# tsai0507/PolishPathPlanning

Hardware: AMD Instinct MI355X
Metric: polishing waypoints/sec for 1M-pt cloud, 256 slices; path L2 err vs ref (higher is better)
Workload: dtype f32; 1 GPU; cfg2_1m_s256; points_per_workpiece=999912, slices=256, waypoints_per_workpiece=25908, workpieces=1, batch_per_gpu=1, parallelism=single GPU, pairing=kd, walk=center_int (connect), dynamic_adjustment=False, handles_taking_turns=3

## Files before the change

### polishpathplanning_amd/csrc/ppp_engine.hip

```cpp
#include "ppp_kernels.h"
#ifdef PPP_SINGLE_TU
#include "ppp_window.h"
#endif
#include "ppp_handle.h"
#include "ppp_gather.h"
#include <atomic>
#include <cerrno>
#include <fcntl.h>
#include <thread>
#include <unistd.h>
#ifndef PPP_NN_HINT_SPACINGS
#define PPP_NN_HINT_SPACINGS 3.0
#endif
#ifndef PPP_SLAB_PTS
#define PPP_SLAB_PTS 832
#endif
#ifndef PPP_PPT8_FROM
#define PPP_PPT8_FROM 500000
#endif
#ifndef WIN_SLICE_WAVES_PER_CU
#define WIN_SLICE_WAVES_PER_CU 16
#endif
#ifndef PPP_WIN_PPT8_FROM
#define PPP_WIN_PPT8_FROM 1200000
// ... 410 lines not shown
static void win_args_throughput(const ppp_handle h, WinArgs &A)
{
    A.NBc = h->win_NBc_thr; A.NB = WIN_CLASSES * A.NBc;
    const float yr = h->h_mx[1] - h->h_mn[1];
    A.yscale = yr > 0.f ? (float)A.NBc / yr : 0.f;
}

static int enqueue_window_gen(ppp_handle h)
{
    WinArgs A = win_args(h);
    const bool thr = win_throughput_launch(h, A.g_slice);
    if (thr) win_args_throughput(h, A);
    const size_t scat_lds = win_scatter_lds_bytes(A.S, h->win_ppt, h->win_scat_threads, h->win_staged);
    if (h->win_scat_threads != WSC_T) {
        const int rcn = with_narrow_scatter(h->win_scat_threads, h->win_ppt, [&](auto ppt, auto st) -> int {
            LAUNCH(h, "k_win_scatter", (k_win_scatter<decltype(ppt)::value, false, decltype(st)::value>), A.g_scatter, decltype(st)::value, scat_lds, A);
            return PPP_OK;
        });
        if (rcn) return rcn;
    }
    else if (h->win_staged && h->win_ppt == 8) LAUNCH(h, "k_win_scatter", (k_win_scatter<8, true>), A.g_scatter, WSC_T, scat_lds, A);
    else if (h->win_staged) LAUNCH(h, "k_win_scatter", (k_win_scatter<4, true>), A.g_scatter, WSC_T, scat_lds, A);
    else if (h->win_ppt == 8) LAUNCH(h, "k_win_scatter", (k_win_scatter<8, false>), A.g_scatter, WSC_T, scat_lds, A);
    else if (h->win_ppt == 2) LAUNCH(h, "k_win_scatter", (k_win_scatter<2, false>), A.g_scatter, WSC_T, scat_lds, A);
    else LAUNCH(h, "k_win_scatter", (k_win_scatter<4, false>), A.g_scatter, WSC_T, scat_lds, A);
    const int T = h->win_threads;
    const size_t lds = win_slice_lds_for(h, A.NBc);
    const int extra = tuning_env("PPP_WIN_NO_VERIFY") ? 0 : 1;
    return with_block_size(T, [&](auto bs) -> int {
        LAUNCH(h, "k_win_slice", k_win_slice<decltype(bs)::value>, A.g_slice + extra, T, lds, A);
        return PPP_OK;
    });
}
static int enqueue_window_finish(ppp_handle h)
{
    const WinArgs A = win_args(h);
    LAUNCH(h, "k_win_finish", k_win_finish, A.g_finish, SMF_T, sizeof(int) * ((size_t)A.nkept + 2), A);
    return PPP_OK;
}

static int make_plan(ppp_handle h)
{
    if (!h->have_cloud) return fail(h, PPP_ERR_ARG, "no cloud set");
    h->pass.withdraw_plan();
    h->drop_graph();
    const int n = (int)h->n;
    int S = h->h_nvalid ? ppp_slice_walk(h->P.walk, h->h_mn[0], h->h_mx[0], h->P.tool_radius, nullptr, 0) : 0;
    if (S >= PPP_WALK_HARD_MAX) return fail(h, PPP_ERR_CAPACITY, "slice walk does not terminate");
    h->sb = std::min(std::max(0, h->P.slice_begin), S);
    h->se = (h->P.slice_end <= 0 || h->P.slice_end > S) ? S : h->P.slice_end;
    h->ranged = S > 0 && (h->sb > 0 || h->se < S);
    h->incl_lo = -INFINITY; h->incl_hi = INFINITY;
    h->n_range = h->h_nvalid;
    if (h->ranged) {
        if (h->sb >= h->se) { h->incl_lo = INFINITY; h->incl_hi = -INFINITY; h->n_range = 0; }
        else {
            std::vector<float> px((size_t)S);
            ppp_slice_walk(h->P.walk, h->h_mn[0], h->h_mx[0], h->P.tool_radius, px.data(), S);
            h->incl_lo = (float)((int)px[h->sb] - 2) - h->P.range_margin;
            h->incl_hi = (float)((int)px[h->se - 1] + 2) + h->P.range_margin;
            const double range = (double)h->h_mx[0] - (double)h->h_mn[0];
            const double part = std::min((double)h->incl_hi, (double)h->h_mx[0]) - std::max((double)h->incl_lo, (double)h->h_mn[0]);
            h->n_range = range > 0 ? (int)std::min((double)h->h_nvalid, std::max(0.0, part / range) * h->h_nvalid * 1.05 + 64) : h->h_nvalid;
        }
    }
    h->use_part = false; h->n_part = 0;
    if (h->part_given) {
        if (!h->ranged && !(h->part_lo == -INFINITY && h->part_hi == INFINITY))
            return fail(h, PPP_ERR_ARG, "a part-only cloud (ppp_set_cloud_part) needs a slice range: set slice_begin / slice_end");
// ... 902 lines not shown
    const SlabGeom G = slab_geom(h);
    const SlabArgs A = slab_args(h, G);
    int rc = enqueue_index(h, G, A);
    if (rc) return rc;
    if (h->P.pairing == PPP_PAIR_KD) {
        LAUNCH(h, "k_slice_kd", k_slice_kd<false>, A.g_slice, G.slice_threads(h->num_cus), G.slice_lds(), A);
        if (h->big_path) LAUNCH(h, "k_slice_kd_arena", k_slice_kd<true>, A.g_slice, SLICE_KD_T, 0, A);
    } else {
        LAUNCH(h, "k_slice", k_slice, A.g_slice, K_SLICE_T, G.brute_lds(), A);
        if (h->big_path) LAUNCH(h, "k_slice_brute_arena", k_slice_brute_arena, A.g_slice, 1024, 0, A);
    }
    if (h->P.dynamic_adjustment) {
        int rc2 = enqueue_dynamic(h);
        if (rc2) return rc2;
    }
    h->pass.gen_enqueued(false);
    if (h->chain_calls) return PPP_OK;
    return enqueue_meta_copy(h);
}

int enqueue_finish(ppp_handle h, const SlabArgs &A)
{
    LAUNCH(h, "k_smooth_solve", k_smooth_solve, A.g_smooth, SMF_T, 0, A);
    return enqueue_meta_copy(h);
}

int ppp_get_path_async(ppp_handle h)
{
    if (!h) return PPP_ERR_ARG;
    HIPCHK(h, hipSetDevice(h->device));
    { int rcs = settle_enqueue_only(h); if (rcs) return rcs; }
    if (!h->pass.gen_done()) return fail(h, PPP_ERR_ARG, "call ppp_gen_path_async first");
    if (h->win_path) {
        int rcw = enqueue_window_finish(h);
        if (rcw) return rcw;
        h->pass.path_enqueued(!h->ranged, true);
        h->pass.meta_will_arrive(MetaAt::pinned());
        return PPP_OK;
    }
    const SlabGeom G = slab_geom(h);
    const SlabArgs A = slab_args(h, G);
    PoseBack PB;
    memset(&PB, 0, sizeof(PB));
    if (h->aligned) {
        if (h->ranged) return fail(h, PPP_ERR_UNSUPPORTED, "Alignment with a slice range");
        if (!h->back || !h->back->pass.index_built()) return fail(h, PPP_ERR_ARG, "aligned cloud without its sensor-frame index");
        PB.sorted4 = h->back->sorted4.p; PB.slab_start = h->back->slab_start.p; PB.slab_xmin = h->back->slab_xmin.p; PB.slab_xmax = h->back->slab_xmax.p;
        PB.m = h->back->meta.p; PB.ytab = h->back->slab_ytab.p;
        for (int r = 0; r < 3; ++r) for (int c = 0; c < 4; ++c) PB.inv[r][c] = h->invTA[r][c];
        LAUNCH(h, "k_pose<aligned>", (k_pose<true, POSE_T>), A.g_pose, G.pose_threads, G.pose_lds, A, PB);
    } else {
        const int rcp = with_block_size(G.pose_threads, [&](auto bs) -> int {
            LAUNCH(h, "k_pose", (k_pose<false, decltype(bs)::value>), A.g_pose, G.pose_threads, G.pose_lds, A, PB);
            return PPP_OK;
        });
        if (rcp) return rcp;
    }
    h->pass.path_enqueued(false, false);
    if (!h->ranged) {
        int rc = enqueue_finish(h, A);
        if (rc) return rc;
        h->pass.path_enqueued(true, false);
        return PPP_OK;
    }
    return enqueue_meta_copy(h);
}

int ppp_finish_path_async(ppp_handle h, const float *pre6_dev, size_t W, const int *counts, size_t nkept)
{
// ... 519 lines not shown
}

int ppp_get_tail_index(ppp_handle h, int *tail, size_t cap, size_t *n)
{
    int rc = ensure_ready(h, true, true);
    if (rc) return rc;
    if (!h->pass.list_final()) return fail(h, PPP_ERR_ARG, NOT_FINAL_MSG);
    rc = map_dev_err(h);
    if (rc) return rc;
    size_t nk = (size_t)h->hmeta.nkept;
    if (n) *n = nk;
    if (tail && cap) {
        size_t k = std::min(cap, nk);
        if (k) HIPCHK(h, copy_sync(h, tail, h->tail.p, k * sizeof(int), hipMemcpyDeviceToHost));
    }
    return PPP_OK;
}

int ppp_get_waypoint_counts(ppp_handle h, int *counts, size_t cap, size_t *nkept)
{
    int rc = ensure_ready(h, true, true);
    if (rc) return rc;
    rc = map_dev_err(h);
    if (rc) return rc;
    size_t nk = (size_t)h->hmeta.nkept;
    if (nkept) *nkept = nk;
    if (counts && cap) {
        size_t k = std::min(cap, nk);
        if (k) HIPCHK(h, copy_sync(h, counts, h->wp_cnt.p, k * sizeof(int), hipMemcpyDeviceToHost));
    }
    return PPP_OK;
}

int ppp_copy_stage_to_device(ppp_handle h, int stage, float *dst_dev, size_t cap, size_t *W)
{
    int rc = ensure_ready(h, true, true);
    if (rc) return rc;
    rc = map_dev_err(h);
    if (rc) return rc;
    const float *src = stage == PPP_STAGE_WP_PRESMOOTH ? h->wp_pre.p : stage == PPP_STAGE_WP_SMOOTHED ? h->wp_smooth.p : nullptr;
    if (!src) return fail(h, PPP_ERR_ARG, "stage must be PPP_STAGE_WP_PRESMOOTH or PPP_STAGE_WP_SMOOTHED");
    if (stage == PPP_STAGE_WP_SMOOTHED && !h->pass.list_final()) return fail(h, PPP_ERR_ARG, NOT_FINAL_MSG);
    size_t w = (size_t)h->hmeta.W;
    if (W) *W = w;
    size_t k = std::min(cap, w);
    if (k && dst_dev) {
        HIPCHK(h, hipMemcpyAsync(dst_dev, src, k * 24, hipMemcpyDeviceToDevice, h->stream));
        HIPCHK(h, hipStreamSynchronize(h->stream));
    }
    return PPP_OK;
}

static int bounds_ready(ppp_handle h)
{
    if (h && h->have_cloud && h->pass.planned() && h->win_path && h->pass.gen_done()) {
        HIPCHK(h, hipSetDevice(h->device));
        return PPP_OK;
    }
    return ensure_index(h);
}

int ppp_minmax(ppp_handle h, float mn[3], float mx[3])
{
    int rc = bounds_ready(h);
    if (rc) return rc;
    rc = fetch_meta(h);
    if (rc) return rc;
    for (int d = 0; d < 3; ++d) { mn[d] = h->hmeta.mn[d]; mx[d] = h->hmeta.mx[d]; }
    return PPP_OK;
}

int ppp_get_slice_positions(ppp_handle h, float *px, size_t cap, size_t *S)
// ... 240 lines not shown
int ppp_nearest(ppp_handle h, const float *q_xyz, size_t k, int *idx)
{
    int rc = index_ready(h, false);
    if (rc) return rc;
    if (!k) return PPP_OK;
    if (!q_xyz || !idx) return fail(h, PPP_ERR_ARG, "bad arguments");
    HIPCHK(h, h->scratch.ensure(k * 16));
    float *dq = (float *)h->scratch.p;
    int *dout = (int *)(dq + 3 * k);
    HIPCHK(h, hipMemcpyAsync(dq, q_xyz, k * 12, hipMemcpyHostToDevice, h->stream));
    LAUNCH(h, "k_nearest_api", k_nearest_api, (unsigned)((k + 63) / 64), 64, 0, h->meta.p, h->sorted4.p, h->slab_start.p, h->slab_xmin.p,
           h->slab_xmax.p, dq, (int)k, dout);
    HIPCHK(h, hipMemcpyAsync(idx, dout, k * 4, hipMemcpyDeviceToHost, h->stream));
    HIPCHK(h, hipStreamSynchronize(h->stream));
    return PPP_OK;
}

static int ensure_stage_lists(ppp_handle h)
{
    if (h->pass.stage_compact() || !h->win_path) return PPP_OK;
    const WinArgs A = win_args(h);
    if (A.nkept > 0) LAUNCH(h, "k_win_gather_stage", k_win_gather_stage, A.nkept, 256, 0, A, h->wp_xyz.p, h->wp_nn.p, h->wp_normal.p);
    h->pass.stages_gathered();
    return PPP_OK;
}

int ppp_get_stage(ppp_handle h, int stage, void *out, size_t cap_bytes, size_t *count)
{
    int rc = ensure_ready(h, true, true);
    if (rc) return rc;
    rc = map_dev_err(h);
    if (rc) return rc;
    if (stage == PPP_STAGE_WP_XYZ || stage == PPP_STAGE_WP_NN || stage == PPP_STAGE_WP_NORMAL) { rc = ensure_stage_lists(h); if (rc) return rc; }
    size_t W = (size_t)h->hmeta.W;
    if (count) *count = W;
    if (!out || !cap_bytes || !W) return PPP_OK;
    const void *src = nullptr;
    size_t elem = 0;
    std::vector<float> tmp;
    switch (stage) {
    case PPP_STAGE_WP_XYZ: {
        std::vector<float4> t4(W);
        HIPCHK(h, copy_sync(h, t4.data(), h->wp_xyz.p, W * 16, hipMemcpyDeviceToHost));
        tmp.resize(3 * W);
        for (size_t i = 0; i < W; ++i) { tmp[3 * i] = t4[i].x; tmp[3 * i + 1] = t4[i].y; tmp[3 * i + 2] = t4[i].z; }
        memcpy(out, tmp.data(), std::min(cap_bytes, W * 12));
        return PPP_OK;
    }
    case PPP_STAGE_WP_NN: src = h->wp_nn.p; elem = 4; break;
    case PPP_STAGE_WP_NORMAL: src = h->wp_normal.p; elem = 16; break;
    case PPP_STAGE_WP_PRESMOOTH: src = h->wp_pre.p; elem = 24; break;
    case PPP_STAGE_WP_SMOOTHED: src = h->wp_smooth.p; elem = 24; break;
    default: return fail(h, PPP_ERR_ARG, "unknown stage");
    }
    HIPCHK(h, copy_sync(h, out, src, std::min(cap_bytes, W * elem), hipMemcpyDeviceToHost));
    return PPP_OK;
}

struct ppp_spline_s {
    int device = 0;
    hipStream_t stream = nullptr;
    size_t n = 0;
    double miny = 0, bigy = 0;
    DevBuf<double> knots;
    DevBuf<double> scratch;
    DevBuf<int> flag;
// ... 197 lines not shown
```

### polishpathplanning_amd/csrc/ppp_handle.h

```cpp
#pragma once
#include "ppp_window_decl.h"
#include "ppp_dynamic.h"
#include "ppp_compact.h"
#include "../../include/ppp_hip.h"
#include <algorithm>
#include <cmath>
#include <cstdlib>
#include <functional>
#include <memory>
#include <string>
#include <vector>

struct RegAcc;
struct FeedRec;

namespace ppp_internal __attribute__((visibility("hidden"))) {

struct KTimer {
    std::string name;
    std::vector<hipEvent_t> e0, e1;
    int used = 0;
};

template <typename T, bool PINNED>
// ... 8 lines not shown
    {
        if (this != &o) { release(); p = o.p; cap = o.cap; o.p = nullptr; o.cap = 0; }
        return *this;
    }
    ~OwnedBuf() { release(); }
    hipError_t ensure(size_t n)
    {
        if (n <= cap && p) return hipSuccess;
        release();
        if (n == 0) n = 1;
        hipError_t e = PINNED ? hipHostMalloc((void **)&p, n * sizeof(T), hipHostMallocDefault) : hipMalloc((void **)&p, n * sizeof(T));
        if (e == hipSuccess) cap = n;
        return e;
    }
    void release() { if (p) (void)(PINNED ? hipHostFree(p) : hipFree(p)); p = nullptr; cap = 0; }
};
template <typename T> using DevBuf = OwnedBuf<T, false>;
template <typename T> using PinBuf = OwnedBuf<T, true>;

struct MetaAt {
    enum Kind { ON_DEMAND , PINNED , BATCH_SLOT  };
    Kind kind = ON_DEMAND;
    std::shared_ptr<PinBuf<DevMeta>> batch;
    size_t slot = 0;
    static MetaAt on_demand() { return MetaAt(); }
    static MetaAt pinned() { MetaAt a; a.kind = PINNED; return a; }
    static MetaAt batch_slot(const std::shared_ptr<PinBuf<DevMeta>> &metas, size_t i) { MetaAt a; a.kind = BATCH_SLOT; a.batch = metas; a.slot = i; return a; }
};

class PassState {
    bool planned_ = false, index_built_ = false, gen_done_ = false, path_done_ = false;
    bool list_final_ = false;
    bool stage_compact_ = true;
    unsigned long long serial_ = 0;
    bool meta_fresh_ = false;
    MetaAt meta_at_;
    hipStream_t pending_stream_ = nullptr;
    void withdraw_results() { index_built_ = false; gen_done_ = false; meta_fresh_ = false; path_done_ = false; list_final_ = false; }

public:
    bool planned() const { return planned_; }
    bool index_built() const { return index_built_; }
    bool gen_done() const { return gen_done_; }
    bool path_done() const { return path_done_; }
    bool list_final() const { return list_final_; }
    bool stage_compact() const { return stage_compact_; }
    unsigned long long serial() const { return serial_; }
    bool meta_fresh() const { return meta_fresh_; }
    bool meta_in_flight() const { return meta_at_.kind != MetaAt::ON_DEMAND; }
    const DevMeta *meta_landing(const DevMeta *handle_block) const
    {
        return (meta_at_.kind == MetaAt::BATCH_SLOT && meta_at_.batch) ? meta_at_.batch->p + meta_at_.slot : handle_block;
    }
    hipStream_t pending_stream() const { return pending_stream_; }

    void withdraw_plan() { planned_ = false; withdraw_results(); }
    void plan_made() { stage_compact_ = true; planned_ = true; withdraw_results(); }
    void cloud_replaced_under_plan() { withdraw_results(); }
    void index_enqueued() { index_built_ = true; }
    void gen_enqueued(bool window) { if (window) stage_compact_ = false; gen_done_ = true; ++serial_; path_done_ = false; }
    void path_enqueued(bool final, bool window) { path_done_ = true; list_final_ = final; if (!window) stage_compact_ = true; }
    void pass_enqueued(bool window, bool final, MetaAt at, hipStream_t carrier = nullptr)
    {
        if (!window) index_built_ = true;
        stage_compact_ = !window;
        gen_done_ = true; ++serial_; path_done_ = true;
        list_final_ = final;
        meta_will_arrive(std::move(at));
        pending_stream_ = carrier;
    }
    void restore_results(bool had_path, bool was_final) { gen_done_ = true; path_done_ = had_path; list_final_ = was_final; }
    void stages_gathered() { stage_compact_ = true; }
    void streams_settled() { pending_stream_ = nullptr; }
    void meta_will_arrive(MetaAt at)
    {
        if (at.kind == MetaAt::BATCH_SLOT) meta_at_ = std::move(at); else meta_at_.kind = at.kind;
        meta_fresh_ = false;
    }
    void meta_stale() { meta_fresh_ = false; }
    void meta_read() { meta_at_.kind = MetaAt::ON_DEMAND; meta_fresh_ = true; }
};

}
using namespace ppp_internal;

struct ppp_handle_s {
    int device = 0;
    hipStream_t stream = nullptr;
    std::string err;
    ppp_params P;
    float vp[3] = {0, 0, 0};
    size_t n = 0;
    bool have_cloud = false;
    PassState pass;
    unsigned long long hn_serial = ~0ull;
    std::vector<int> hn_off;
    std::vector<float> hn_xyz;
    DevBuf<int> pack_tab;
    DevBuf<float> pack_out;
    int max_lds = 65536;
    int num_cus = 256;

    int B = 1, slab_cap = 4096, S_cap = 1, capb = 2048, W_cap = 1, node_cap = 1;
    int knot_cap = 2048, stage_cap = POSE_STAGE_CAP, tab_slabs = 8, pose_threads = POSE_T, cnt_est = 1;
    float pose_pad = 8.f;
// ... 366 lines not shown
```

### polishpathplanning_amd/csrc/ppp_window.h

```cpp
#pragma once
#include "ppp_kernels.h"
#include "ppp_window_decl.h"

template <int PPT, bool STAGED, int T = WSC_T>
__device__ __forceinline__ void win_scatter_body(const WinArgs &A, const int bx)
{
    extern __shared__ __attribute__((aligned(16))) int s_dyn[];
    float *s_px = (float *)s_dyn;
    int *s_cnt = s_dyn + A.S;
    __shared__ int s_scr[17];
    __shared__ float s_mn[3][T / 64], s_mx[3][T / 64];
    __shared__ int s_n[T / 64];
    const int S = A.S, n = A.n;
    const int i0 = bx * (PPT * (int)blockDim.x);
    STAMP_BEGIN();
    float4 p[PPT];
#pragma unroll
    for (int k = 0; k < PPT; ++k) {
        const int i = i0 + threadIdx.x + k * (int)blockDim.x;
        if (i < n) p[k] = make_float4(A.X[i], A.Y[i], A.Z[i], __int_as_float(A.idmap ? A.idmap[i] : i));
        else p[k] = make_float4(NAN, 0.f, 0.f, 0.f);
    }
    for (int s = threadIdx.x; s < S; s += blockDim.x) { s_px[s] = A.plan_px[s]; s_cnt[s] = 0; }
    if (bx == 0 && threadIdx.x == 0) {
// ... 896 lines not shown
            for (int d = 0; d < 3; ++d) if (rmn[d] != R.fin.mn[d] || rmx[d] != R.fin.mx[d]) bad = 1;
            if (c != R.fin.cnt || R.S != A.S || __float_as_int(R.pad) != __float_as_int(A.pad)) bad = 1;
        } else {
            for (int d = 0; d < 3; ++d) if (rmn[d] != A.plan_mn[d] || rmx[d] != A.plan_mx[d]) bad = 1;
            if (c != A.plan_nvalid) bad = 1;
        }
        int S = c ? slice_walk_device(P.walk, rmn[0], rmx[0], P.tool_radius, s_px, A.S, s_front, 2048) : 0;
        if (S != A.S) bad = 1;
        for (int d = 0; d < 3; ++d) { m->mn[d] = rmn[d]; m->mx[d] = rmx[d]; m->mn_ord[d] = f2ord(rmn[d]); m->mx_ord[d] = f2ord(rmx[d]); }
        m->n_valid = c;
        m->S = S > A.S ? A.S : S;
        m->first_kept = P.drop_ends ? 1 : 0;
        { const int Sc = S > A.S ? A.S : S, nk = P.drop_ends ? Sc - 2 : Sc; m->nkept = nk < 0 ? 0 : nk; }
        m->sb = A.sb; m->se = A.se;
        m->incl_lo = P.incl_lo; m->incl_hi = P.incl_hi;
        s_S = S > A.S ? A.S : S;
        if (bad) s_bad = 1;
    }
    __syncthreads();
    const int S = s_S;
    int bad = 0;
    for (int s = tid; s < S; s += T) {
        const float v = s_px[s];
        if (v != A.plan_px[s]) bad = 1;
        const int position = (int)v;
        A.px[s] = v; A.lo[s] = (float)(-2 + position); A.hi[s] = (float)(2 + position);
    }
    if (bad) s_bad = 1;
    __syncthreads();
    if (tid == 0 && s_bad) win_flag(m, WIN_FLAG_STALE);
}

#define META_PUT(ptr, val) __hip_atomic_store((ptr), (val), __ATOMIC_RELAXED, __HIP_MEMORY_SCOPE_AGENT)
__device__ __forceinline__ void win_finish_body(const WinArgs &A, const int bx)
{
    extern __shared__ __attribute__((aligned(16))) int s_off[];
    __shared__ float s_x[3][SMF_M];
    __shared__ int s_scan[17];
    __shared__ int s_run, s_short, s_last, s_err;
    __shared__ double s_rp[SMF_END];
    __shared__ double s_e[2][3];
    DevMeta *m = A.m;
    const DevParams &P = A.P;
    const int nk = A.nkept, tid = (int)threadIdx.x;
    if (tid == 0) { s_err = m->err | m->win_flag; s_run = 0; s_short = 0; }
    __syncthreads();
    if (s_err) return;
    const int res_i = (int)P.rpy_resolution;
    for (int base = 0; base < nk; base += blockDim.x) {
        const int k2 = base + tid;
        int c2 = 0;
        if (k2 < nk) {
            const int s2 = k2 + A.first_kept;
            if (s2 >= A.sb && s2 < A.se) c2 = A.wp_cnt[k2];
        }
        int tot;
        const int pre = block_exscan_w(c2, s_scan, &tot);
        const int run = s_run;
        if (k2 < nk) {
            s_off[k2] = run + pre;
            if (P.rpy_resolution > 2 && c2 <= res_i) s_short = 1;
        }
        __syncthreads();
        if (tid == 0) s_run = run + tot;
        __syncthreads();
    }
    const int W = s_run;
    if (tid == 0) s_off[nk] = W;
    __syncthreads();
    if (W > A.W_cap) { if (bx == 0 && tid == 0) { set_err(m, DERR_CAPACITY, -1); META_PUT(&m->W, 0); } return; }
    if (bx == 0) {
        for (int k2 = tid; k2 < nk; k2 += blockDim.x) {
            A.wp_off[k2] = s_off[k2]; A.tail[k2] = s_off[k2 + 1] - 1;
            const int s2 = k2 + A.first_kept;
            if (s2 < A.sb || s2 >= A.se) A.wp_cnt[k2] = 0;
        }
        if (tid == 0) { A.wp_off[nk] = W; META_PUT(&m->W, W); META_PUT(&m->any_short, s_short); META_PUT(&m->sweeps, 0); META_PUT(&m->smooth_done, 0); }
    }
    const int ntiles = smooth_tiles(W);
    const int tile = bx;
    if (W == 0 || tile >= ntiles) return;
    auto slice_of = [&](int g) {
        int kk = (int)(((long long)g * (long long)nk) / (long long)W);
        kk = kk < 0 ? 0 : (kk > nk - 1 ? nk - 1 : kk);
        int steps = 0;
        while (kk > 0 && s_off[kk] > g && steps < 6) { --kk; ++steps; }
        while (kk < nk - 1 && s_off[kk + 1] <= g && steps < 6) { ++kk; ++steps; }
        if (steps >= 6) { int lo = 0, hi = nk - 1; while (lo < hi) { const int mid = (lo + hi + 1) >> 1; if (s_off[mid] <= g) lo = mid; else hi = mid - 1; } kk = lo; }
        return kk;
    };
    auto row_of = [&](int g) { const int kk = slice_of(g); return (size_t)kk * A.stride + (size_t)(g - s_off[kk]); };
    const double wd = 0.65, ws = 1 - wd, dg = wd + 2 * ws;
    const double r = (dg - sqrt(dg * dg - 4 * ws * ws)) / (2 * ws), c = wd / (dg - 2 * ws * r);
    const int t0 = tile * SMF_T;
    const int base = t0 - SMF_K;
    const bool solve = A.finish && P.smooth && W > 2;
    const int g = t0 + tid;
    int kk = 0;
    size_t rowbase = 0;
    float p[6] = {0.f, 0.f, 0.f, 0.f, 0.f, 0.f};
    if (g < W) {
        kk = slice_of(g);
        rowbase = (size_t)kk * A.stride - (size_t)s_off[kk];
#pragma unroll
        for (int d = 0; d < 6; ++d) p[d] = A.wps_pre[6 * (rowbase + g) + d];
    }
    if (A.finish) {
        const bool src = g >= 1 && g <= W - 2;
        for (int j = 0; j < 3; ++j) s_x[j][tid + SMF_K] = src ? p[j] : 0.f;
        if (tid < 2 * SMF_K) {
            const int l = tid < SMF_K ? tid : SMF_T + tid;
            const int g2 = base + l;
            const bool src2 = g2 >= 1 && g2 <= W - 2;
            size_t row = 0;
            if (src2) row = row_of(g2);
            for (int j = 0; j < 3; ++j) s_x[j][l] = src2 ? A.wps_pre[6 * row + j] : 0.f;
        }
    }
    const bool in_order = A.finish && P.rpy_resolution > 2 && s_short;
    const bool copy2 = A.finish && A.out2 != nullptr && W <= A.out2_cap;
    if (A.finish && A.out2 != nullptr && W > A.out2_cap && tile == 0 && tid == 0) set_err(m, DERR_CAPACITY, -1);
    const bool near_end = solve && (t0 < SMF_END || t0 + SMF_T - 1 > W - 1 - SMF_END);
    if (near_end) {
        if (tid < SMF_END) s_rp[tid] = smooth_rpow(r, tid);
        const int j = tid >> 6, lane = tid & 63;
        if (j < 3) {
            const int kq = (lane & 31) + 1;
            const int gq = lane < 32 ? kq : W - 1 - kq;
            double v = (gq >= 1 && gq <= W - 2) ? (double)A.wps_pre[6 * row_of(gq) + j] * smooth_rpow(r, kq) : 0.0;
            for (int o = 16; o > 0; o >>= 1) v += __shfl_xor(v, o, 64);
            if ((lane & 31) == 0) s_e[lane >> 5][j] = (double)A.wps_pre[6 * row_of(lane < 32 ? 0 : W - 1) + j] - c * v;
        }
    }
    __syncthreads();
    if (g < W) {
#pragma clang fp contract(on)
        for (int d = 0; d < 6; ++d) A.wp_pre[6 * (size_t)g + d] = p[d];
        if (A.finish) {
            if (solve) {
                const int l = g - base;
                double y[3];
#pragma unroll
                for (int j = 0; j < 3; ++j) {
                    double acc = (double)s_x[j][l - SMF_K] + (double)s_x[j][l + SMF_K];
#pragma unroll 8
                    for (int q = SMF_K - 1; q >= 1; --q) acc = ((double)s_x[j][l - q] + (double)s_x[j][l + q]) + r * acc;
                    y[j] = c * ((double)s_x[j][l] + r * acc);
                }
                if (near_end) {
                    const double D = W - 1 < SMF_END ? s_rp[W - 1] : 0.0;
                    const double r0 = g < SMF_END ? s_rp[g] : 0.0, r1 = W - 1 - g < SMF_END ? s_rp[W - 1 - g] : 0.0;
                    const double det = 1.0 - D * D;
#pragma unroll
                    for (int j = 0; j < 3; ++j) {
                        const double e0 = s_e[0][j], e1 = s_e[1][j];
                        const double Aa = (e0 - D * e1) / det, Bb = (e1 - D * e0) / det;
                        y[j] = y[j] + (Aa * r0 + Bb * r1);
                    }
                }
                if (g >= 1 && g <= W - 2) { p[0] = (float)y[0]; p[1] = (float)y[1]; p[2] = (float)y[2]; }
            }
            for (int d = 0; d < 6; ++d) A.wp_smooth[6 * (size_t)g + d] = p[d];
            if (!in_order) {
                if (P.rpy_resolution > 2) {
                    const int res = res_i;
                    const int p0 = s_off[kk], tl = s_off[kk + 1] - 1;
                    const int nfull = (tl - p0) / res;
                    const int lastkey = p0 + nfull * res;
                    const int rr = g - p0;
                    const float *src = A.wps_pre + 6 * rowbase;
                    if (g > lastkey) {
                        for (int D = 3; D < 6; ++D) p[D] = src[6 * (size_t)lastkey + D];
                    } else if (rr % res != 0) {
                        const int pre = p0 + (rr / res) * res, last = pre + res, wi = g - pre;
                        for (int D = 3; D < 6; D++) {
                            const float a = src[6 * (size_t)last + D], bb = src[6 * (size_t)pre + D];
                            double dr;
                            if (a * bb >= 0) {
                                dr = (double)((a - bb) / res);
                            } else {
                                double no1, no2;
                                if (a < 0) { no2 = bb; no1 = 2 * M_PI + a; }
                                else { no2 = 2 * M_PI + bb; no1 = a; }
                                dr = (double)fabsf(a - bb) < fabs(no1 - no2) ? (double)(a - bb) : (no1 - no2);
                                dr /= res;
                            }
                            float v = bb;
                            for (int q = 1; q <= wi; ++q) v = (float)(dr + v);
                            p[D] = v;
                        }
                    }
                    for (int D = 3; D < 6; ++D) p[D] = (double)p[D] > M_PI ? (float)((double)p[D] - 2 * M_PI) : p[D];
                }
                float R[3][3];
                rot_zyx(p[3], p[4], p[5], R);
                const float ee[3] = {0.f, 0.f, -P.ee_length};
                float t[3];
                for (int i = 0; i < 3; ++i) t[i] = R[i][0] * ee[0] + R[i][1] * ee[1] + R[i][2] * ee[2] + p[i] * 1.f;
                p[0] = t[0]; p[1] = t[1]; p[2] = t[2];
            }
            for (int d = 0; d < 6; ++d) A.wp_out[6 * (size_t)g + d] = p[d];
            if (copy2 && !in_order) for (int d = 0; d < 6; ++d) A.out2[6 * (size_t)g + d] = p[d];
        }
    }
    if (in_order) {
        __threadfence();
        __syncthreads();
        if (tid == 0) s_last = atomicAdd(&m->emit_ticket, 1) == ntiles - 1;
        __syncthreads();
        if (s_last) {
            __threadfence();
            if (tid == 0) { finish_list_in_order(m, P, A.tail, A.wp_out); m->emit_ticket = 0; }
            __threadfence();
            __syncthreads();
            if (copy2) for (size_t i = tid; i < 6 * (size_t)W; i += blockDim.x) A.out2[i] = A.wp_out[i];
        }
    }
}

__global__ void __launch_bounds__(256) k_win_gather_stage(WinArgs A, float4 *wp_xyz, int *wp_nn, float4 *wp_normal)
{
    const int k = blockIdx.x;
    if (k >= A.nkept) return;
    const int s = k + A.first_kept;
    if (s < A.sb || s >= A.se) return;
    const int off = A.wp_off[k], cnt = A.wp_cnt[k];
    for (int t = threadIdx.x; t < cnt; t += blockDim.x) {
        const size_t slot = (size_t)k * A.stride + t;
        wp_xyz[off + t] = A.wps_xyz[slot];
        wp_nn[off + t] = A.wps_nn[slot];
        wp_normal[off + t] = A.wps_normal[slot];
    }
}



__device__ __forceinline__ void win_census_point(float x, const float *__restrict__ px, int S, float px0, float inv_step, float pad,
                                                 int *cw, int *ce, int *cr)
// ... 111 lines not shown
}
template <int TMAX>
__global__ void __launch_bounds__(TMAX) k_win_slice_b(const WinArgs *__restrict__ mem)
{
    const WinArgs &A = mem[blockIdx.y];
    if ((int)blockIdx.x > A.g_slice) return;
    if ((int)blockIdx.x == A.g_slice) { win_verify_body(A); return; }
    win_slice_body<TMAX>(A, blockIdx.x);
}
__device__ __forceinline__ void win_publish_meta(const WinArgs &A)
{
    if (!A.meta_host) return;
    __shared__ int s_lastw;
    __syncthreads();
    if (threadIdx.x == 0) {
        __builtin_amdgcn_s_waitcnt(0);
        const int grp = (int)blockIdx.x % WIN_FIN_GROUPS;
        const int members = (A.g_finish - grp + WIN_FIN_GROUPS - 1) / WIN_FIN_GROUPS;
        int last = 0;
        if (__hip_atomic_fetch_add(A.fin_ticket + 1 + grp, 1, __ATOMIC_RELAXED, __HIP_MEMORY_SCOPE_AGENT) == members - 1) {
            __hip_atomic_store(A.fin_ticket + 1 + grp, 0, __ATOMIC_RELAXED, __HIP_MEMORY_SCOPE_AGENT);
            const int groups = A.g_finish < WIN_FIN_GROUPS ? A.g_finish : WIN_FIN_GROUPS;
            last = __hip_atomic_fetch_add(A.fin_ticket, 1, __ATOMIC_RELAXED, __HIP_MEMORY_SCOPE_AGENT) == groups - 1;
        }
        s_lastw = last;
    }
    __syncthreads();
    if (!s_lastw) return;
    const int *src = (const int *)A.m;
    int *dst = (int *)A.meta_host;
    for (int q = threadIdx.x; q < (int)(sizeof(DevMeta) / sizeof(int)); q += blockDim.x) dst[q] = __hip_atomic_load(src + q, __ATOMIC_RELAXED, __HIP_MEMORY_SCOPE_AGENT);
    if (threadIdx.x == 0) __hip_atomic_store(A.fin_ticket, 0, __ATOMIC_RELAXED, __HIP_MEMORY_SCOPE_AGENT);
}
__global__ void __launch_bounds__(SMF_T) k_win_finish(WinArgs A) { win_finish_body(A, blockIdx.x); win_publish_meta(A); }
__global__ void __launch_bounds__(SMF_T) k_win_finish_b(const WinArgs *__restrict__ mem)
{
    const WinArgs &A = mem[blockIdx.y];
    if ((int)blockIdx.x >= A.g_finish) return;
    win_finish_body(A, blockIdx.x);
    win_publish_meta(A);
}
```

### polishpathplanning_amd/csrc/ppp_window_decl.h

```cpp
#pragma once
#include "ppp_kernels.h"

enum { WIN_FLAG_OVERFLOW = 1,
       WIN_FLAG_REACH = 2,
       WIN_FLAG_STALE = 4 };
__device__ inline void win_flag(DevMeta *m, int why) { atomicOr(&m->win_flag, why); }

#define WIN_CLASSES 5
#ifndef WIN_CNT_STRIDE
#define WIN_CNT_STRIDE 1
#endif
#ifndef WIN_EMAX
#define WIN_EMAX 8
#endif
#ifndef WIN_CE
#define WIN_CE 4
#endif

struct WinArgs {
    DevMeta *m;
    DevParams P;
    const float *X, *Y, *Z;
    const int *idmap;
    int n;
    const float *plan_px;
    int S, sb, se, first_kept, nkept;
    float pad, px0, inv_step, y0, yscale;
    float plan_mn[3], plan_mx[3];
    int plan_nvalid;
    int capw, cap_el, NB, NBc, stride, W_cap, node_cap;
    int rec_lds;
    int g_scatter, g_slice, g_finish;
    int finish;
    int *win_cnt;
    float4 *win_pts;
    MinMaxPart *win_part;
    float *px, *lo, *hi;
    float *node_x, *node_y, *node_z;
    int *node_start, *node_cnt, *band_cnt;
    int *wp_cnt, *wp_off, *tail;
    float4 *wps_xyz, *wps_normal;
    float4 *wps_rec;
    int *wps_nn;
    float *wps_pre;
    float *wp_pre, *wp_smooth, *wp_out, *out2;
    int out2_cap;
    DevMeta *meta_host;
    int *fin_ticket;
    const PlanAuto *plan_rec;
};

__host__ __device__ inline size_t win_slice_lds_bytes(int capw, int cap_el, int NB)
{
    return (size_t)capw * 16 + (((size_t)NB + 1) * 4 + 15) / 16 * 16 + (size_t)cap_el * 16 + 16;
}

#ifndef WSC_T
#define WSC_T 1024
#endif
__host__ __device__ inline size_t win_scatter_lds_bytes(int S, int ppt, int threads, bool staged)
{
    return staged ? (size_t)12 * S + 16 + (size_t)18 * ppt * threads : (size_t)8 * S;
}
#ifndef WSL_T
#define WSL_T 1024
#endif
#define WIN_FIN_GROUPS 32
#define WIN_S_MAX 8192
#define WIN_AUTO_SCAP 4096

template <int PPT, bool STAGED, int T = WSC_T> __global__ void k_win_scatter(WinArgs A);
template <int PPT, bool STAGED, int T = WSC_T> __global__ void k_win_scatter_b(const WinArgs *__restrict__ mem);
template <int TMAX> __global__ void k_win_slice(WinArgs A);
template <int TMAX> __global__ void k_win_slice_b(const WinArgs *__restrict__ mem);
__global__ void k_win_finish(WinArgs A);
__global__ void k_win_finish_b(const WinArgs *__restrict__ mem);
__global__ void k_win_gather_stage(WinArgs A, float4 *wp_xyz, int *wp_nn, float4 *wp_normal);
template <bool IN_LDS>
__global__ void k_win_census(const float *__restrict__ X, int n, const float *__restrict__ px, int S, float px0, float inv_step, float pad,
                             int *cnt_win, int *cnt_el, int *cnt_er);
__global__ void k_win_census_auto(const float *__restrict__ X, int n, const float *px, const PlanAuto *plan, float inv_step, int *cnt, int *ticket,
                                  PlanAuto *plan_host, float *px_host, int *census_host);
```

Baseline: 960.4 million waypoints/s.

## Defer intermediate stage list writes in window finish and restructure its scan and loads

The window finish kernel no longer writes the presmooth and smoothed waypoint lists on the default internal path. An on-demand kernel, k_win_stage_lists, rebuilds them only when a caller requests those stages, tracked by a staleness flag in the pass state. The kernel also uses a single-pass 4-per-thread scan when the kept slice count is small, and issues all its global loads (halo, keyframe rows, end terms) up front. This reduces memory writes and barriers in the finish pass, at the cost of more state-tracking complexity and a second launch whenever stages are queried.

```diff
diff --git a/polishpathplanning_amd/csrc/ppp_engine.hip b/polishpathplanning_amd/csrc/ppp_engine.hip
--- a/polishpathplanning_amd/csrc/ppp_engine.hip
+++ b/polishpathplanning_amd/csrc/ppp_engine.hip
@@ -466,9 +466,10 @@
         return PPP_OK;
     });
 }
-static int enqueue_window_finish(ppp_handle h)
-{
-    const WinArgs A = win_args(h);
+static int enqueue_window_finish(ppp_handle h, bool finish_lists)
+{
+    WinArgs A = win_args(h);
+    A.stage_lists = finish_lists ? 1 : 0;
     LAUNCH(h, "k_win_finish", k_win_finish, A.g_finish, SMF_T, sizeof(int) * ((size_t)A.nkept + 2), A);
     return PPP_OK;
 }
@@ -1437,9 +1438,10 @@
     { int rcs = settle_enqueue_only(h); if (rcs) return rcs; }
     if (!h->pass.gen_done()) return fail(h, PPP_ERR_ARG, "call ppp_gen_path_async first");
     if (h->win_path) {
-        int rcw = enqueue_window_finish(h);
+        const bool finish_lists = h->ranged || !h->internal;
+        int rcw = enqueue_window_finish(h, finish_lists);
         if (rcw) return rcw;
-        h->pass.path_enqueued(!h->ranged, true);
+        h->pass.path_enqueued(!h->ranged, true, finish_lists);
         h->pass.meta_will_arrive(MetaAt::pinned());
         return PPP_OK;
     }
@@ -2025,12 +2027,22 @@
     return PPP_OK;
 }
 
+static int ensure_finish_lists(ppp_handle h)
+{
+    if (!h->pass.finish_lists_stale() || !h->win_path) return PPP_OK;
+    const WinArgs A = win_args(h);
+    LAUNCH(h, "k_win_stage_lists", k_win_stage_lists, A.g_finish, SMF_T, sizeof(int) * ((size_t)A.nkept + 2), A);
+    h->pass.finish_lists_made();
+    return PPP_OK;
+}
+
 int ppp_copy_stage_to_device(ppp_handle h, int stage, float *dst_dev, size_t cap, size_t *W)
 {
     int rc = ensure_ready(h, true, true);
     if (rc) return rc;
     rc = map_dev_err(h);
     if (rc) return rc;
+    if (stage == PPP_STAGE_WP_PRESMOOTH || stage == PPP_STAGE_WP_SMOOTHED) { rc = ensure_finish_lists(h); if (rc) return rc; }
     const float *src = stage == PPP_STAGE_WP_PRESMOOTH ? h->wp_pre.p : stage == PPP_STAGE_WP_SMOOTHED ? h->wp_smooth.p : nullptr;
     if (!src) return fail(h, PPP_ERR_ARG, "stage must be PPP_STAGE_WP_PRESMOOTH or PPP_STAGE_WP_SMOOTHED");
     if (stage == PPP_STAGE_WP_SMOOTHED && !h->pass.list_final()) return fail(h, PPP_ERR_ARG, NOT_FINAL_MSG);
@@ -2337,6 +2349,7 @@
     rc = map_dev_err(h);
     if (rc) return rc;
     if (stage == PPP_STAGE_WP_XYZ || stage == PPP_STAGE_WP_NN || stage == PPP_STAGE_WP_NORMAL) { rc = ensure_stage_lists(h); if (rc) return rc; }
+    if (stage == PPP_STAGE_WP_PRESMOOTH || stage == PPP_STAGE_WP_SMOOTHED) { rc = ensure_finish_lists(h); if (rc) return rc; }
     size_t W = (size_t)h->hmeta.W;
     if (count) *count = W;
     if (!out || !cap_bytes || !W) return PPP_OK;
diff --git a/polishpathplanning_amd/csrc/ppp_handle.h b/polishpathplanning_amd/csrc/ppp_handle.h
--- a/polishpathplanning_amd/csrc/ppp_handle.h
+++ b/polishpathplanning_amd/csrc/ppp_handle.h
@@ -64,6 +64,7 @@
     bool planned_ = false, index_built_ = false, gen_done_ = false, path_done_ = false;
     bool list_final_ = false;
     bool stage_compact_ = true;
+    bool finish_lists_stale_ = false;
     unsigned long long serial_ = 0;
     bool meta_fresh_ = false;
     MetaAt meta_at_;
@@ -77,6 +78,7 @@
     bool path_done() const { return path_done_; }
     bool list_final() const { return list_final_; }
     bool stage_compact() const { return stage_compact_; }
+    bool finish_lists_stale() const { return finish_lists_stale_; }
     unsigned long long serial() const { return serial_; }
     bool meta_fresh() const { return meta_fresh_; }
     bool meta_in_flight() const { return meta_at_.kind != MetaAt::ON_DEMAND; }
@@ -91,11 +93,16 @@
     void cloud_replaced_under_plan() { withdraw_results(); }
     void index_enqueued() { index_built_ = true; }
     void gen_enqueued(bool window) { if (window) stage_compact_ = false; gen_done_ = true; ++serial_; path_done_ = false; }
-    void path_enqueued(bool final, bool window) { path_done_ = true; list_final_ = final; if (!window) stage_compact_ = true; }
+    void path_enqueued(bool final, bool window, bool finish_lists = true)
+    {
+        path_done_ = true; list_final_ = final; finish_lists_stale_ = !finish_lists;
+        if (!window) stage_compact_ = true;
+    }
     void pass_enqueued(bool window, bool final, MetaAt at, hipStream_t carrier = nullptr)
     {
         if (!window) index_built_ = true;
         stage_compact_ = !window;
+        finish_lists_stale_ = window && final;
         gen_done_ = true; ++serial_; path_done_ = true;
         list_final_ = final;
         meta_will_arrive(std::move(at));
@@ -103,6 +110,7 @@
     }
     void restore_results(bool had_path, bool was_final) { gen_done_ = true; path_done_ = had_path; list_final_ = was_final; }
     void stages_gathered() { stage_compact_ = true; }
+    void finish_lists_made() { finish_lists_stale_ = false; }
     void streams_settled() { pending_stream_ = nullptr; }
     void meta_will_arrive(MetaAt at)
     {
diff --git a/polishpathplanning_amd/csrc/ppp_window.h b/polishpathplanning_amd/csrc/ppp_window.h
--- a/polishpathplanning_amd/csrc/ppp_window.h
+++ b/polishpathplanning_amd/csrc/ppp_window.h
@@ -952,6 +952,7 @@
 }
 
 #define META_PUT(ptr, val) __hip_atomic_store((ptr), (val), __ATOMIC_RELAXED, __HIP_MEMORY_SCOPE_AGENT)
+template <bool ONDEMAND>
 __device__ __forceinline__ void win_finish_body(const WinArgs &A, const int bx)
 {
     extern __shared__ __attribute__((aligned(16))) int s_off[];
@@ -963,33 +964,59 @@
     DevMeta *m = A.m;
     const DevParams &P = A.P;
     const int nk = A.nkept, tid = (int)threadIdx.x;
-    if (tid == 0) { s_err = m->err | m->win_flag; s_run = 0; s_short = 0; }
-    __syncthreads();
-    if (s_err) return;
     const int res_i = (int)P.rpy_resolution;
-    for (int base = 0; base < nk; base += blockDim.x) {
-        const int k2 = base + tid;
-        int c2 = 0;
-        if (k2 < nk) {
-            const int s2 = k2 + A.first_kept;
-            if (s2 >= A.sb && s2 < A.se) c2 = A.wp_cnt[k2];
-        }
+    int W;
+    if (nk <= 4 * SMF_T) {
+        int c4[4];
+#pragma unroll
+        for (int u = 0; u < 4; ++u) {
+            const int k2 = 4 * tid + u, s2 = k2 + A.first_kept;
+            c4[u] = (k2 < nk && s2 >= A.sb && s2 < A.se) ? A.wp_cnt[k2] : 0;
+        }
+        if (tid == 0) { s_err = m->err | m->win_flag; s_short = 0; }
         int tot;
-        const int pre = block_exscan_w(c2, s_scan, &tot);
-        const int run = s_run;
-        if (k2 < nk) {
-            s_off[k2] = run + pre;
-            if (P.rpy_resolution > 2 && c2 <= res_i) s_short = 1;
-        }
-        __syncthreads();
-        if (tid == 0) s_run = run + tot;
-        __syncthreads();
-    }
-    const int W = s_run;
+        int pre = block_exscan_w(c4[0] + c4[1] + c4[2] + c4[3], s_scan, &tot);
+        if (s_err) return;
+        bool shrt = false;
+#pragma unroll
+        for (int u = 0; u < 4; ++u) {
+            const int k2 = 4 * tid + u;
+            if (k2 < nk) {
+                s_off[k2] = pre;
+                pre += c4[u];
+                if (c4[u] <= res_i) shrt = true;
+            }
+        }
+        if (P.rpy_resolution > 2 && shrt) s_short = 1;
+        W = tot;
+    } else {
+        if (tid == 0) { s_err = m->err | m->win_flag; s_run = 0; s_short = 0; }
+        __syncthreads();
+        if (s_err) return;
+        for (int base = 0; base < nk; base += blockDim.x) {
+            const int k2 = base + tid;
+            int c2 = 0;
+            if (k2 < nk) {
+                const int s2 = k2 + A.first_kept;
+                if (s2 >= A.sb && s2 < A.se) c2 = A.wp_cnt[k2];
+            }
+            int tot;
+            const int pre = block_exscan_w(c2, s_scan, &tot);
+            const int run = s_run;
+            if (k2 < nk) {
+                s_off[k2] = run + pre;
+                if (P.rpy_resolution > 2 && c2 <= res_i) s_short = 1;
+            }
+            __syncthreads();
+            if (tid == 0) s_run = run + tot;
+            __syncthreads();
+        }
+        W = s_run;
+    }
     if (tid == 0) s_off[nk] = W;
     __syncthreads();
-    if (W > A.W_cap) { if (bx == 0 && tid == 0) { set_err(m, DERR_CAPACITY, -1); META_PUT(&m->W, 0); } return; }
-    if (bx == 0) {
+    if (W > A.W_cap) { if (!ONDEMAND && bx == 0 && tid == 0) { set_err(m, DERR_CAPACITY, -1); META_PUT(&m->W, 0); } return; }
+    if (!ONDEMAND && bx == 0) {
         for (int k2 = tid; k2 < nk; k2 += blockDim.x) {
             A.wp_off[k2] = s_off[k2]; A.tail[k2] = s_off[k2 + 1] - 1;
             const int s2 = k2 + A.first_kept;
@@ -1015,58 +1042,97 @@
     const int t0 = tile * SMF_T;
     const int base = t0 - SMF_K;
     const bool solve = A.finish && P.smooth && W > 2;
+    const bool in_order = A.finish && P.rpy_resolution > 2 && s_short;
+    const bool lists = ONDEMAND || A.stage_lists || !A.finish || in_order;
+    const bool near_end = solve && (t0 < SMF_END || t0 + SMF_T - 1 > W - 1 - SMF_END);
     const int g = t0 + tid;
     int kk = 0;
     size_t rowbase = 0;
-    float p[6] = {0.f, 0.f, 0.f, 0.f, 0.f, 0.f};
     if (g < W) {
         kk = slice_of(g);
         rowbase = (size_t)kk * A.stride - (size_t)s_off[kk];
-#pragma unroll
-        for (int d = 0; d < 6; ++d) p[d] = A.wps_pre[6 * (rowbase + g) + d];
-    }
+    }
+    const bool halo = A.finish && tid < 2 * SMF_K;
+    const int hl = tid < SMF_K ? tid : SMF_T + tid;
+    bool hsrc = false;
+    size_t hrow = 0;
+    if (halo) {
+        const int g2 = base + hl;
+        hsrc = g2 >= 1 && g2 <= W - 2;
+        if (hsrc) hrow = row_of(g2);
+    }
+    int kmode = 0, wi = 0;
+    size_t krow_a = 0, krow_b = 0;
+    if (!ONDEMAND && g < W && A.finish && !in_order && P.rpy_resolution > 2) {
+        const int res = res_i;
+        const int p0 = s_off[kk], tl = s_off[kk + 1] - 1;
+        const int nfull = (tl - p0) / res;
+        const int lastkey = p0 + nfull * res;
+        const int rr = g - p0;
+        if (g > lastkey) { kmode = 1; krow_b = rowbase + (size_t)lastkey; }
+        else if (rr % res != 0) {
+            const int pre = p0 + (rr / res) * res, last = pre + res;
+            kmode = 2; krow_b = rowbase + (size_t)pre; krow_a = rowbase + (size_t)last; wi = g - pre;
+        }
+    }
+    const int ej = tid >> 6, lane = tid & 63;
+    const bool eterm = near_end && ej < 3;
+    const int kq = (lane & 31) + 1;
+    bool qsrc = false;
+    size_t qrow = 0, erow = 0;
+    if (eterm) {
+        const int gq = lane < 32 ? kq : W - 1 - kq;
+        qsrc = gq >= 1 && gq <= W - 2;
+        if (qsrc) qrow = row_of(gq);
+        if ((lane & 31) == 0) erow = row_of(lane < 32 ? 0 : W - 1);
+    }
+    typedef const __attribute__((address_space(1))) float *gfloat_p;
+    const gfloat_p wps = (gfloat_p)A.wps_pre;
+    const size_t orow = g < W ? rowbase + (size_t)g : 0;
+    const int ejc = ej < 3 ? ej : 0;
+    float p[6], hx[3], ka[3], kb[3];
+#pragma unroll
+    for (int d = 0; d < 6; ++d) p[d] = wps[6 * orow + d];
+#pragma unroll
+    for (int j = 0; j < 3; ++j) hx[j] = wps[6 * hrow + j];
+#pragma unroll
+    for (int D = 3; D < 6; ++D) kb[D - 3] = wps[6 * krow_b + D];
+#pragma unroll
+    for (int D = 3; D < 6; ++D) ka[D - 3] = wps[6 * krow_a + D];
+    const float qv = wps[6 * qrow + ejc], ev = wps[6 * erow + ejc];
     if (A.finish) {
         const bool src = g >= 1 && g <= W - 2;
         for (int j = 0; j < 3; ++j) s_x[j][tid + SMF_K] = src ? p[j] : 0.f;
-        if (tid < 2 * SMF_K) {
-            const int l = tid < SMF_K ? tid : SMF_T + tid;
-            const int g2 = base + l;
-            const bool src2 = g2 >= 1 && g2 <= W - 2;
-            size_t row = 0;
-            if (src2) row = row_of(g2);
-            for (int j = 0; j < 3; ++j) s_x[j][l] = src2 ? A.wps_pre[6 * row + j] : 0.f;
-        }
-    }
-    const bool in_order = A.finish && P.rpy_resolution > 2 && s_short;
-    const bool copy2 = A.finish && A.out2 != nullptr && W <= A.out2_cap;
-    if (A.finish && A.out2 != nullptr && W > A.out2_cap && tile == 0 && tid == 0) set_err(m, DERR_CAPACITY, -1);
-    const bool near_end = solve && (t0 < SMF_END || t0 + SMF_T - 1 > W - 1 - SMF_END);
+        const int hslot = halo ? hl : tid + SMF_K;
+        for (int j = 0; j < 3; ++j) s_x[j][hslot] = halo ? (hsrc ? hx[j] : 0.f) : (src ? p[j] : 0.f);
+    }
+    const bool copy2 = !ONDEMAND && A.finish && A.out2 != nullptr && W <= A.out2_cap;
+    if (!ONDEMAND && A.finish && A.out2 != nullptr && W > A.out2_cap && tile == 0 && tid == 0) set_err(m, DERR_CAPACITY, -1);
     if (near_end) {
         if (tid < SMF_END) s_rp[tid] = smooth_rpow(r, tid);
-        const int j = tid >> 6, lane = tid & 63;
-        if (j < 3) {
-            const int kq = (lane & 31) + 1;
-            const int gq = lane < 32 ? kq : W - 1 - kq;
-            double v = (gq >= 1 && gq <= W - 2) ? (double)A.wps_pre[6 * row_of(gq) + j] * smooth_rpow(r, kq) : 0.0;
+        if (ej < 3) {
+            double v = qsrc ? (double)qv * smooth_rpow(r, kq) : 0.0;
             for (int o = 16; o > 0; o >>= 1) v += __shfl_xor(v, o, 64);
-            if ((lane & 31) == 0) s_e[lane >> 5][j] = (double)A.wps_pre[6 * row_of(lane < 32 ? 0 : W - 1) + j] - c * v;
+            if ((lane & 31) == 0) s_e[lane >> 5][ej] = (double)ev - c * v;
         }
     }
     __syncthreads();
     if (g < W) {
 #pragma clang fp contract(on)
-        for (int d = 0; d < 6; ++d) A.wp_pre[6 * (size_t)g + d] = p[d];
+        if (lists) for (int d = 0; d < 6; ++d) A.wp_pre[6 * (size_t)g + d] = p[d];
         if (A.finish) {
             if (solve) {
                 const int l = g - base;
-                double y[3];
-#pragma unroll
-                for (int j = 0; j < 3; ++j) {
-                    double acc = (double)s_x[j][l - SMF_K] + (double)s_x[j][l + SMF_K];
+                double acc[3], y[3];
+#pragma unroll
+                for (int j = 0; j < 3; ++j) acc[j] = (double)s_x[j][l - SMF_K] + (double)s_x[j][l + SMF_K];
 #pragma unroll 8
-                    for (int q = SMF_K - 1; q >= 1; --q) acc = ((double)s_x[j][l - q] + (double)s_x[j][l + q]) + r * acc;
-                    y[j] = c * ((double)s_x[j][l] + r * acc);
+                for (int q = SMF_K - 1; q >= 1; --q) {
+#pragma unroll
+                    for (int j = 0; j < 3; ++j) acc[j] = ((double)s_x[j][l - q] + (double)s_x[j][l + q]) + r * acc[j];
                 }
+#pragma unroll
+                for (int j = 0; j < 3; ++j) y[j] = c * ((double)s_x[j][l] + r * acc[j]);
                 if (near_end) {
                     const double D = W - 1 < SMF_END ? s_rp[W - 1] : 0.0;
                     const double r0 = g < SMF_END ? s_rp[g] : 0.0, r1 = W - 1 - g < SMF_END ? s_rp[W - 1 - g] : 0.0;
@@ -1080,50 +1146,46 @@
                 }
                 if (g >= 1 && g <= W - 2) { p[0] = (float)y[0]; p[1] = (float)y[1]; p[2] = (float)y[2]; }
             }
-            for (int d = 0; d < 6; ++d) A.wp_smooth[6 * (size_t)g + d] = p[d];
-            if (!in_order) {
-                if (P.rpy_resolution > 2) {
-                    const int res = res_i;
-                    const int p0 = s_off[kk], tl = s_off[kk + 1] - 1;
-                    const int nfull = (tl - p0) / res;
-                    const int lastkey = p0 + nfull * res;
-                    const int rr = g - p0;
-                    const float *src = A.wps_pre + 6 * rowbase;
-                    if (g > lastkey) {
-                        for (int D = 3; D < 6; ++D) p[D] = src[6 * (size_t)lastkey + D];
-                    } else if (rr % res != 0) {
-                        const int pre = p0 + (rr / res) * res, last = pre + res, wi = g - pre;
-                        for (int D = 3; D < 6; D++) {
-                            const float a = src[6 * (size_t)last + D], bb = src[6 * (size_t)pre + D];
-                            double dr;
-                            if (a * bb >= 0) {
-                                dr = (double)((a - bb) / res);
-                            } else {
-                                double no1, no2;
-                                if (a < 0) { no2 = bb; no1 = 2 * M_PI + a; }
-                                else { no2 = 2 * M_PI + bb; no1 = a; }
-                                dr = (double)fabsf(a - bb) < fabs(no1 - no2) ? (double)(a - bb) : (no1 - no2);
-                                dr /= res;
+            if (lists) for (int d = 0; d < 6; ++d) A.wp_smooth[6 * (size_t)g + d] = p[d];
+            if (!ONDEMAND) {
+                if (!in_order) {
+                    if (P.rpy_resolution > 2) {
+                        const int res = res_i;
+                        if (kmode == 1) {
+                            for (int D = 3; D < 6; ++D) p[D] = kb[D - 3];
+                        } else if (kmode == 2) {
+                            for (int D = 3; D < 6; D++) {
+                                const float a = ka[D - 3], bb = kb[D - 3];
+                                double dr;
+                                if (a * bb >= 0) {
+                                    dr = (double)((a - bb) / res);
+                                } else {
+                                    double no1, no2;
+                                    if (a < 0) { no2 = bb; no1 = 2 * M_PI + a; }
+                                    else { no2 = 2 * M_PI + bb; no1 = a; }
+                                    dr = (double)fabsf(a - bb) < fabs(no1 - no2) ? (double)(a - bb) : (no1 - no2);
+                                    dr /= res;
+                                }
+                                float v = bb;
+                                for (int q = 1; q <= wi; ++q) v = (float)(dr + v);
+                                p[D] = v;
                             }
-                            float v = bb;
-                            for (int q = 1; q <= wi; ++q) v = (float)(dr + v);
-                            p[D] = v;
                         }
+                        for (int D = 3; D < 6; ++D) p[D] = (double)p[D] > M_PI ? (float)((double)p[D] - 2 * M_PI) : p[D];
                     }
-                    for (int D = 3; D < 6; ++D) p[D] = (double)p[D] > M_PI ? (float)((double)p[D] - 2 * M_PI) : p[D];
+                    float R[3][3];
+                    rot_zyx(p[3], p[4], p[5], R);
+                    const float ee[3] = {0.f, 0.f, -P.ee_length};
+                    float t[3];
+                    for (int i = 0; i < 3; ++i) t[i] = R[i][0] * ee[0] + R[i][1] * ee[1] + R[i][2] * ee[2] + p[i] * 1.f;
+                    p[0] = t[0]; p[1] = t[1]; p[2] = t[2];
                 }
-                float R[3][3];
-                rot_zyx(p[3], p[4], p[5], R);
-                const float ee[3] = {0.f, 0.f, -P.ee_length};
-                float t[3];
-                for (int i = 0; i < 3; ++i) t[i] = R[i][0] * ee[0] + R[i][1] * ee[1] + R[i][2] * ee[2] + p[i] * 1.f;
-                p[0] = t[0]; p[1] = t[1]; p[2] = t[2];
-            }
-            for (int d = 0; d < 6; ++d) A.wp_out[6 * (size_t)g + d] = p[d];
-            if (copy2 && !in_order) for (int d = 0; d < 6; ++d) A.out2[6 * (size_t)g + d] = p[d];
-        }
-    }
-    if (in_order) {
+                for (int d = 0; d < 6; ++d) A.wp_out[6 * (size_t)g + d] = p[d];
+                if (copy2 && !in_order) for (int d = 0; d < 6; ++d) A.out2[6 * (size_t)g + d] = p[d];
+            }
+        }
+    }
+    if (!ONDEMAND && in_order) {
         __threadfence();
         __syncthreads();
         if (tid == 0) s_last = atomicAdd(&m->emit_ticket, 1) == ntiles - 1;
@@ -1301,11 +1363,12 @@
     for (int q = threadIdx.x; q < (int)(sizeof(DevMeta) / sizeof(int)); q += blockDim.x) dst[q] = __hip_atomic_load(src + q, __ATOMIC_RELAXED, __HIP_MEMORY_SCOPE_AGENT);
     if (threadIdx.x == 0) __hip_atomic_store(A.fin_ticket, 0, __ATOMIC_RELAXED, __HIP_MEMORY_SCOPE_AGENT);
 }
-__global__ void __launch_bounds__(SMF_T) k_win_finish(WinArgs A) { win_finish_body(A, blockIdx.x); win_publish_meta(A); }
+__global__ void __launch_bounds__(SMF_T) k_win_finish(WinArgs A) { win_finish_body<false>(A, blockIdx.x); win_publish_meta(A); }
 __global__ void __launch_bounds__(SMF_T) k_win_finish_b(const WinArgs *__restrict__ mem)
 {
     const WinArgs &A = mem[blockIdx.y];
     if ((int)blockIdx.x >= A.g_finish) return;
-    win_finish_body(A, blockIdx.x);
+    win_finish_body<false>(A, blockIdx.x);
     win_publish_meta(A);
 }
+__global__ void __launch_bounds__(SMF_T) k_win_stage_lists(WinArgs A) { win_finish_body<true>(A, blockIdx.x); }
diff --git a/polishpathplanning_amd/csrc/ppp_window_decl.h b/polishpathplanning_amd/csrc/ppp_window_decl.h
--- a/polishpathplanning_amd/csrc/ppp_window_decl.h
+++ b/polishpathplanning_amd/csrc/ppp_window_decl.h
@@ -32,6 +32,7 @@
     int rec_lds;
     int g_scatter, g_slice, g_finish;
     int finish;
+    int stage_lists;
     int *win_cnt;
     float4 *win_pts;
     MinMaxPart *win_part;
@@ -75,6 +76,7 @@
 template <int TMAX> __global__ void k_win_slice_b(const WinArgs *__restrict__ mem);
 __global__ void k_win_finish(WinArgs A);
 __global__ void k_win_finish_b(const WinArgs *__restrict__ mem);
+__global__ void k_win_stage_lists(WinArgs A);
 __global__ void k_win_gather_stage(WinArgs A, float4 *wp_xyz, int *wp_nn, float4 *wp_normal);
 template <bool IN_LDS>
 __global__ void k_win_census(const float *__restrict__ X, int n, const float *__restrict__ px, int S, float px0, float inv_step, float pad,
```

Result: faster. 974.9 million waypoints/s, median of 6 (+1.5%).
